# gavrissh/training-operator

Hardware: AMD Instinct MI355X
Metric: job×node fit evals/sec + gang placements/sec, 1M-node inventory, 1/2/4/8 GPUs (higher is better)
Workload: dtype int64

## Files before the change

training-operator_amd/csrc/pe_ctx.h:

```cpp
#pragma once

#include <hip/hip_runtime.h>
#include <rccl/rccl.h>

#include <immintrin.h>
#include <pthread.h>
#include <sched.h>

#include <algorithm>
#include <atomic>
#include <cstdlib>
#include <cstring>
#include <exception>
#include <functional>
#include <memory>
#include <mutex>
#include <new>
#include <stdexcept>
#include <string>
#include <thread>
#include <vector>

#include "pe_hostx.h"
#include "pe_kernels.h"
// ... 226 lines not shown
  std::thread comm_abort;
  std::unique_ptr<pe::Resolver> resolver;
  pe_allgather_fn exchange = nullptr;
  void* exchange_user = nullptr;
  void* zc_hx = nullptr;
  bool zc_ok = false;
  int topk = 256, window_groups = 112;
  bool pipeline = true;
  int64_t window_pods = 1024;
  int64_t max_nodes = 0;
  std::string gpu_name, err;
  hipStream_t stream = nullptr;
  int64_t n_total = 0, begin = 0, end = 0, Ns = 0, stride = 0;
  bool loaded = false;
  std::vector<pe::NodeState, pe::HugeAlloc<pe::NodeState>> m_nodes, m_nodes0;
  DevBuf<int64_t> res0, res;
  DevBuf<uint32_t> labels;
  DevBuf<int32_t> island;
  DevBuf<pe::NodeUpd> n_upd;
  int64_t fit_J = 0, fit_Jp = 0, Wn = 0, Wt = 0;
  bool fit_uploaded = false;
  DevBuf<ReqRec> fit_jobs;
  DevBuf<pe::ReqRec32> fit_jobs32;
  DevBuf<int32_t> res32;
  bool fit32 = false;
  int fit_shift[pe::D] = {0, 0, 0, 0};
  int fit_path = 0;
  pe::LdsSpec lds{};
  int lds_W = 4;
  int lds_shape[4] = {0, 0, 0, 0};
  int64_t lds_nblk = 0, lds_R = 1, lds_Tpad = 0, lds_npad = 0, lds_pitch = 0;
  DevBuf<pe::LdsSpec> lds_spec_d;
  DevBuf<int64_t> lds_vals;
  DevBuf<uint16_t> lds_codes;
  DevBuf<uint32_t> lds_ranks, lds_aux, lds_slots;
  DevBuf<uint32_t> lds_rows;
  int num_cu = 256;
  int fit_path_mask = PATHS_ALL;
  pe::PlaneSpec plane{};
  int64_t pl_nblk = 0;
  bool pl_rows = true;
  int64_t pl_R = 1;
  int64_t pl_pitch = 0;
  struct PlaneSet {
    pe::PlaneSpec spec;
    int64_t J, R, Jr, off;
  };
  std::vector<PlaneSet> pl_sets;
  DevBuf<pe::PlaneSpec> pl_specs_d;
  DevBuf<int64_t> pl_meta_d;
  std::vector<int64_t> pl_cnt_row;
  int64_t pl_counts_n = 0;
  DevBuf<uint32_t> planes;
  DevBuf<uint64_t> plane_jobs;
  pe::CodeSpec code{};
  int64_t code_Jp = 0, node_stride = 0;
  DevBuf<int64_t> code_vals;
  DevBuf<uint32_t> code_needs, code_jobs, code_x;
  DevBuf<uint64_t> mask;
  DevBuf<unsigned long long> counts;
  HostBuf<unsigned long long> h_counts;
  HostBuf<uint8_t> a_stage, a_outh;
  DevBuf<uint8_t> a_dstage;
  hipStream_t a_h2d = nullptr;
  std::vector<hipEvent_t> a_ev_h2d;
  HostBuf<int64_t> a_segoff;
  HostBuf<uint32_t> a_flag;
// ... 267 lines not shown
```

training-operator_amd/csrc/pe_engine.cpp:

```cpp
#include <hip/hip_runtime.h>
#include <rccl/rccl.h>

#include <immintrin.h>
#include <pthread.h>
#include <sched.h>

#include <algorithm>
#include <condition_variable>
#include <atomic>
#include <chrono>
#include <exception>
#include <functional>
#include <thread>
#include <cstdio>
#include <cstdlib>
#include <cstring>
#include <memory>
#include <mutex>
#include <new>
#include <numeric>
#include <string>
#include <unordered_map>
#include <vector>

#include "pe_ctx.h"
#include "pe_hostx.h"
#include "pe_kernels.h"
#include "pe_resolver.h"
#include "placement.h"

namespace {

double rccl_init_timeout_ms() {
  const char* e = std::getenv("PE_RCCL_INIT_TIMEOUT_S");
  const double s = e ? std::atof(e) : 120.0;
  return (s > 0 ? s : 120.0) * 1e3;
}

ncclComm_t comm_init_bounded(int device, int world, const ncclUniqueId& id, int rank, double timeout_ms) {
  struct State {
    std::mutex m;
    std::condition_variable cv;
    bool done = false, abandoned = false;
    ncclResult_t r = ncclSuccess;
    ncclComm_t comm = nullptr;
  };
  auto st = std::make_shared<State>();
  std::thread([st, device, world, id, rank] {
    (void)hipSetDevice(device);
    ncclComm_t c = nullptr;
    const ncclResult_t r = ncclCommInitRank(&c, world, id, rank);
    std::lock_guard<std::mutex> lk(st->m);
    if (st->abandoned) {
      if (r == ncclSuccess && c) (void)ncclCommDestroy(c);
      return;
    }
    st->r = r;
    st->comm = c;
    st->done = true;
    st->cv.notify_all();
// ... 1560 lines not shown
    const double t = (double)rounds * (0.02 + 1.0 / (double)r);
    if (t < best_t - 1e-9) {
      best_t = t;
      R = r;
    }
  }
  if (const char* ev = std::getenv("PE_LDS_R")) R = std::max<int64_t>(1, std::atoll(ev));
  const int64_t Tmax = ((n_jobs + R - 1) / R + 15) / 16;
  const int64_t Tpad = round_up(std::max<int64_t>(Tmax, 1), 16);
  std::vector<uint16_t> jc((size_t)n_jobs * pe::LD_CODE, 0);
  parallel_for(n_jobs, [&](int64_t j0, int64_t j1) {
  for (int64_t j = j0; j < j1; ++j) {
    uint16_t* c = jc.data() + (size_t)j * pe::LD_CODE;
    for (int i = 0; i < sp.nf; ++i) {
      const int64_t rank = (int64_t)bd.rank[fdim[i]][j] + 1;
      const int o = pe::lds_field_off(i, shape[0], shape[1], shape[2]);
      if (sp.L[i] == 1) {
        c[o] = (uint16_t)(sp.pbase[i][0] + rank - 1);
      } else {
        int64_t x = rank;
        for (int k = 0; k < sp.L[i]; ++k) {
          const int64_t digit = sp.mod[i][k] ? x % sp.mod[i][k] : x;
          x = sp.mod[i][k] ? x / sp.mod[i][k] : 0;
          c[o + k] = (uint16_t)(sp.pbase[i][k] + digit);
        }
      }
    }
    int64_t xc = 0;
    for (int x = 0; x < sp.nx; ++x) xc += (int64_t)bd.rank[fdim[sp.nf + x]][j] * sp.xstride[x];
    c[pe::lds_need_slot(shape[0], shape[1], shape[2], shape[3])] =
        (uint16_t)(sp.need_pbase + bd.rank[4][j] * sp.xprod + xc);
  }
  });
  std::vector<uint16_t> codes((size_t)(R * 16 * Tpad * pe::LD_CODE), 0);
  std::vector<uint32_t> rows((size_t)(R * 16 * Tpad), ~0u);
  {
    int64_t pos = 0;
    for (int64_t v = 0; v < R * 16; ++v) {
      const int64_t r = v / 16, w = v % 16, j0 = r + R * w;
      const int64_t T = j0 < n_jobs ? (n_jobs - j0 + 16 * R - 1) / (16 * R) : 0;
      for (int64_t t = 0; t < T; ++t, ++pos) {
        const uint32_t j = (uint32_t)(j0 + 16 * R * t);
        std::memcpy(codes.data() + (size_t)((v * Tpad + t) * pe::LD_CODE), jc.data() + (size_t)j * pe::LD_CODE,
                    pe::LD_CODE * 2);
        rows[(size_t)(v * Tpad + t)] = j;
      }
    }
    if (pos != n_jobs) raise(PE_EINVAL, "lds: run lengths do not cover the batch");
  }
  if (std::getenv("PE_LDS_DEBUG")) {
    std::fprintf(stderr, "lds: W %d nblk %lld R %lld planes %d need %d fold %d cross %d x %d |", W, (long long)nblk,
                 (long long)R, sp.nplanes, sp.nneed, sp.nfold, sp.nx, sp.xprod);
    for (int i = 0; i < sp.nf; ++i)
      std::fprintf(stderr, " dim %d m %lld L %d B %u", sp.dim[i], (long long)sp.m[i], sp.L[i], sp.mod[i][0]);
    std::fprintf(stderr, "\n");
  }
  ctx->lds = sp;
  ctx->lds_W = W;
  for (int i = 0; i < 4; ++i) ctx->lds_shape[i] = shape[i];
  ctx->lds_nblk = nblk;
  ctx->lds_R = R;
  ctx->lds_Tpad = Tpad;
  hipchk(ctx->lds_slots.ensure((size_t)R * 16 * Tpad + (size_t)ctx->lds_nblk), "alloc count slots");
  hipchk(ctx->lds_rows.ensure((size_t)R * 16 * Tpad), "alloc count rows");
  hipchk(hipMemcpyAsync(ctx->lds_rows.p, rows.data(), rows.size() * 4, hipMemcpyHostToDevice, ctx->stream),
         "H2D lds rows");
  ctx->lds_npad = nblk * S;
  ctx->lds_pitch = nblk * S / 64;
  hipchk(ctx->lds_spec_d.ensure(1), "alloc lds spec");
  hipchk(ctx->lds_vals.ensure(std::max<size_t>(allv.size(), 1)), "alloc lds vals");
  hipchk(ctx->lds_codes.ensure(codes.size()), "alloc lds codes");
  hipchk(ctx->lds_ranks.ensure((size_t)std::max(sp.nf + sp.nx, 1) * ctx->lds_npad), "alloc lds ranks");
  hipchk(ctx->lds_aux.ensure((size_t)2 * ctx->lds_npad), "alloc lds aux");
  hipchk(hipMemcpyAsync(ctx->lds_spec_d.p, &ctx->lds, sizeof(pe::LdsSpec), hipMemcpyHostToDevice, ctx->stream),
         "H2D lds spec");
  if (!allv.empty())
    hipchk(hipMemcpyAsync(ctx->lds_vals.p, allv.data(), allv.size() * 8, hipMemcpyHostToDevice, ctx->stream),
           "H2D lds vals");
  hipchk(hipMemcpyAsync(ctx->lds_codes.p, codes.data(), codes.size() * 2, hipMemcpyHostToDevice, ctx->stream),
         "H2D lds codes");
  hipchk(hipStreamSynchronize(ctx->stream), "sync lds upload");
  return true;
}

static void fit_upload(pe_ctx* ctx, int64_t n_jobs, const int64_t* req, const uint32_t* need) {
  if (n_jobs < 0) raise(PE_EINVAL, "n_jobs < 0");
  if (!ctx->loaded) raise(PE_ESTATE, "no inventory loaded");
  if (n_jobs > 0) {
    need_ptr(req, "req");
    check_req(req, n_jobs, "req");
  }
  const int64_t Jp = round_up(std::max<int64_t>(n_jobs, 1), pe::FM_JT);
  ctx->fit_J = n_jobs;
  ctx->fit_Jp = Jp;
  ctx->Wn = (ctx->Ns + 63) / 64;
  ctx->Wt = (ctx->Wn + 3) / 4;
  const bool planes_ok = ctx->fit_path_mask & PATH_PLANES;
  ctx->fit_path = -1;
  if (n_jobs > 0 && (ctx->fit_path_mask & (PATH_PLANES | PATH_LDS | PATH_CODED))) {
    BatchDict bd;
    build_dict(bd, n_jobs, req, need);
    if (planes_ok && build_planes(ctx, n_jobs, bd, false)) ctx->fit_path = 3;
    else if ((ctx->fit_path_mask & PATH_LDS) && build_lds(ctx, n_jobs, bd)) ctx->fit_path = 4;
    else if (planes_ok && build_planes(ctx, n_jobs, bd, true)) ctx->fit_path = 3;
    else if ((ctx->fit_path_mask & PATH_CODED) && build_codes(ctx, n_jobs, bd)) ctx->fit_path = 2;
  }
  if (ctx->fit_path < 0) {
    bool use32 = true;
    for (int d = 0; d < pe::D && use32; ++d) {
      int64_t mx = 0, orv = 0;
      for (int64_t j = 0; j < n_jobs; ++j) {
        mx = std::max(mx, req[j * pe::D + d]);
// ... 42 lines not shown
                                                 : (size_t)Jp * std::max<int64_t>(ctx->Wt, 1) * 4;
  static const unsigned mask_flags = std::getenv("PE_MASK_CONTIG") ? hipDeviceMallocContiguous : 0u;
  hipchk(ctx->mask.ensure(mask_words, mask_flags), "alloc fit mask");
  const int64_t n_counts = std::max<int64_t>(Jp, ctx->fit_path == 3 ? ctx->pl_counts_n : 0);
  hipchk(ctx->counts.ensure(n_counts + (ctx->fit_path == 3 ? ctx->pl_nblk : 0)), "alloc fit counts");
  hipchk(ctx->h_counts.ensure(n_counts), "alloc pinned counts");
  hipchk(hipStreamSynchronize(ctx->stream), "sync fit upload");
  ctx->fit_uploaded = true;
}

static void fit_run(pe_ctx* ctx) {
  if (!ctx->fit_uploaded) raise(PE_ESTATE, "pe_jobs_upload first");
  const int64_t J = ctx->fit_J;
  const bool encode_zeroes = ctx->fit_path == 3 && ctx->pl_sets.empty() && J > 0 && ctx->Ns > 0 && ctx->pl_nblk > 0;
  if (!encode_zeroes)
    hipchk(hipMemsetAsync(ctx->counts.p, 0, ctx->counts.n * sizeof(unsigned long long), ctx->stream), "memset counts");
  if (J == 0 || ctx->Ns == 0) return;
  const int64_t waves_y = (J + pe::FM_JT - 1) / pe::FM_JT;
  const int64_t want_x = std::max<int64_t>(1, (16384 + waves_y - 1) / waves_y);
  int64_t tpw = (ctx->Ns + 256 * want_x - 1) / (256 * want_x);
  tpw = std::min<int64_t>(16, std::max<int64_t>(1, tpw));
  if (ctx->fit_path == 4) {
    hipchk(hipMemsetAsync(ctx->lds_slots.p, 0, ((size_t)ctx->lds_R * 16 * ctx->lds_Tpad + ctx->lds_nblk) * 4, ctx->stream),
           "memset count slots");
    hipchk(pe::launch_node_ranks(ctx->stream, ctx->res.p, ctx->stride, ctx->labels.p, ctx->Ns, ctx->lds_npad,
                                 ctx->lds_spec_d.p, ctx->lds_vals.p, ctx->lds_ranks.p, ctx->lds_aux.p),
           "launch node_ranks");
    hipchk(pe::launch_fit_mask_lds(ctx->stream, ctx->lds_W, ctx->lds_shape, ctx->lds_spec_d.p, ctx->lds.nplanes,
                                   ctx->lds_ranks.p,
                                   ctx->lds_npad, ctx->lds_aux.p, ctx->lds_nblk, ctx->lds_codes.p, J,
                                   ctx->lds_R, ctx->lds_Tpad, ctx->lds_pitch * 8,
                                   reinterpret_cast<uint8_t*>(ctx->mask.p), ctx->lds_slots.p,
                                   std::getenv("PE_FIT_STATIC") ? nullptr
                                                                : ctx->lds_slots.p + (size_t)ctx->lds_R * 16 * ctx->lds_Tpad),
           "launch fit_mask_lds");
    hipchk(pe::launch_lds_counts(ctx->stream, ctx->lds_slots.p, ctx->lds_rows.p, ctx->lds_R * 16 * ctx->lds_Tpad,
                                 ctx->counts.p),
           "launch lds_counts");
    ctx->stats.fit_runs_lds += 1;
  } else if (ctx->fit_path == 3) {
    if (!ctx->pl_sets.empty()) {
      const int ns = (int)ctx->pl_sets.size();
      hipchk(pe::launch_encode_planes_sets(ctx->stream, ctx->res.p, ctx->stride, ctx->labels.p, ctx->Ns, ctx->pl_nblk,
                                           ctx->pl_specs_d.p, ns, ctx->planes.p),
             "launch encode_planes_sets");
      hipchk(pe::launch_fit_mask_planes_sets(ctx->stream, ctx->planes.p, ctx->pl_nblk, ctx->plane_jobs.p,
                                             ctx->pl_meta_d.p, ns, ctx->pl_sets[0].R,
                                             reinterpret_cast<uint32_t*>(ctx->mask.p), ctx->counts.p, ctx->pl_pitch),
             "launch fit_mask_planes_sets");
      ctx->stats.fit_runs_planes += 1;
      ctx->stats.fit_runs_sets += 1;
      ctx->stats.fit_evals += J * ctx->Ns;
      return;
    }
    hipchk(pe::launch_encode_planes(ctx->stream, ctx->res.p, ctx->stride, ctx->labels.p, ctx->Ns, ctx->pl_nblk,
                                    ctx->plane, ctx->pl_specs_d.p, ctx->planes.p, ctx->counts.p, ctx->counts.n),
           "launch encode_planes");
    if (ctx->pl_rows) {
      unsigned long long* const units = std::getenv("PE_FIT_STATIC") ? nullptr : ctx->counts.p + ctx->pl_counts_n;
      hipchk(pe::launch_fit_mask_planes_rows(ctx->stream, ctx->planes.p, ctx->pl_nblk, ctx->plane_jobs.p, J, ctx->pl_R,
                                             reinterpret_cast<uint32_t*>(ctx->mask.p), ctx->counts.p, ctx->pl_pitch,
                                             units),
             "launch fit_mask_planes_rows");
    } else {
      const int64_t ranges = std::max<int64_t>(1, (16384 + ctx->pl_nblk - 1) / ctx->pl_nblk);
      const int64_t jpw = std::max<int64_t>(64, (J + ranges - 1) / ranges);
      hipchk(pe::launch_fit_mask_planes(ctx->stream, ctx->planes.p, ctx->pl_nblk, ctx->plane_jobs.p, J, jpw,
// ... 187 lines not shown
```

training-operator_amd/csrc/pe_kernels.h:

```cpp
#pragma once
#include <hip/hip_runtime.h>
#include <stdint.h>

namespace pe {

constexpr int D = 4;
constexpr uint64_t SCORE_MAX = (1ull << 40) - 1;
constexpr uint64_t NO_KEY = ~0ull;
constexpr int64_t NEVER = INT64_MIN;

struct alignas(64) ReqRec {
  int64_t q[D];
  uint32_t need;
  uint32_t pad_[7];
};
static_assert(sizeof(ReqRec) == 64, "ReqRec must be 64 B");

struct alignas(32) ReqRec32 {
  int32_t q[D];
  uint32_t need;
  uint32_t pad_[3];
};
static_assert(sizeof(ReqRec32) == 32, "ReqRec32 must be 32 B");

// ... 133 lines not shown
constexpr int LD_NEED_SLOT = 15;
__host__ __device__ constexpr int lds_field_off(int fi, int n4, int n3, int n2) {
  return fi <= n4                ? 4 * fi
         : fi <= n4 + n3         ? 4 * n4 + 3 * (fi - n4)
         : fi <= n4 + n3 + n2    ? 4 * n4 + 3 * n3 + 2 * (fi - n4 - n3)
                                 : 4 * n4 + 3 * n3 + 2 * n2 + (fi - n4 - n3 - n2);
}
__host__ __device__ constexpr int lds_need_slot(int n4, int n3, int n2, int n1) {
  return 4 * n4 + 3 * n3 + 2 * n2 + n1;
}
constexpr int LD_THREADS = 1024;
struct LdsSpec {
  int32_t nf;
  int32_t dim[LD_MAXF];
  int32_t L[LD_MAXF];
  uint32_t div[LD_MAXF][LD_MAXL];
  uint32_t mod[LD_MAXF][LD_MAXL];
  int32_t pbase[LD_MAXF][LD_MAXL];
  int32_t vlo[LD_MAXF][LD_MAXL];
  int32_t nv[LD_MAXF][LD_MAXL];
  int32_t nneed, need_pbase, nplanes, nfold;
  int32_t nx, xprod;
  int32_t xstride[LD_MAXF];
  uint32_t needs[LD_MAXNEED];
  int32_t fold_dim[D];
  int64_t fold_val[D];
  int64_t voff[LD_MAXF];
  int64_t m[LD_MAXF];
};
hipError_t launch_node_ranks(hipStream_t s, const int64_t* res, int64_t stride, const uint32_t* labels, int64_t Ns,
                             int64_t npad, const LdsSpec* spec, const int64_t* vals, uint32_t* ranks, uint32_t* aux);
hipError_t launch_fit_mask_lds(hipStream_t s, int W, const int shape[4], const LdsSpec* spec, int nplanes,
                               const uint32_t* ranks, int64_t npad, const uint32_t* aux, int64_t nblk,
                               const uint16_t* codes, int64_t J, int64_t R, int64_t Tpad, int64_t pitch_bytes,
                               uint8_t* mask, uint32_t* slots, uint32_t* units = nullptr);
hipError_t launch_lds_counts(hipStream_t s, const uint32_t* slots, const uint32_t* rows, int64_t nslots,
                             unsigned long long* counts);

hipError_t launch_prep_nodes(hipStream_t s, const int64_t* res, int64_t stride, int64_t Ns, uint64_t id_base,
                             uint64_t* kn, uint32_t* lo );
hipError_t launch_scan(hipStream_t s, const int64_t* res, int64_t stride, const uint32_t* labels, const uint64_t* kn,
                       const uint32_t* lo, int64_t Ns, uint64_t id_base, const ReqRec* groups, int Wg, uint64_t* cand,
                       int32_t* cnt, uint64_t* bound, int nwaves);

hipError_t launch_merge(hipStream_t s, const uint64_t* cand, const int32_t* cnt, const uint64_t* bound,
                        int nwaves, int K, uint8_t* out, int Wg);

constexpr int WK_ROUND = 1024;
constexpr int WK_MAXR = 16384;
constexpr uint64_t WK_INVALID = ~0ull;
#ifndef WK_MULTI
#define WK_MULTI 2
#endif
#ifndef WK_MULTI_AFTER
#define WK_MULTI_AFTER 1
#endif
struct WalkIndex {
  uint64_t* sk;
  int64_t* sr;
  uint32_t* sl;
  uint32_t* pos;
  uint64_t* rmin;
  int64_t* rmax;
  uint32_t* ror;
  int32_t* ovl;
  int32_t* ovl_n;
  uint32_t* in_ovl;
  uint32_t* ovl_idx;
// ... 241 lines not shown
```

training-operator_amd/csrc/pe_lds.hip:

```cpp
#include "pe_lds_kernel.h"

namespace pe {

__global__ __launch_bounds__(256) void node_ranks_kernel(const int64_t* __restrict__ res, int64_t stride,
                                                         const uint32_t* __restrict__ labels, int64_t Ns, int64_t npad,
                                                         const LdsSpec* __restrict__ spp,
                                                         const int64_t* __restrict__ vals, uint32_t* __restrict__ ranks,
                                                         uint32_t* __restrict__ aux) {
  const LdsSpec& sp = *spp;
  const int64_t n = (int64_t)blockIdx.x * blockDim.x + threadIdx.x;
  if (n >= npad) return;
  const bool real = n < Ns;
  uint32_t ok = real ? 1u : 0u;
  for (int i = 0; i < sp.nfold; ++i) ok &= real && res[sp.fold_dim[i] * stride + n] >= sp.fold_val[i];
  aux[n] = ok;
  aux[npad + n] = real ? labels[n] : 0u;
  for (int f = 0; f < sp.nf + sp.nx; ++f) {
    uint32_t R = 0;
    if (real) {
      const int64_t x = res[sp.dim[f] * stride + n];
      const int64_t* v = vals + sp.voff[f];
      int64_t lo = 0, hi = sp.m[f];
      while (lo < hi) {
        const int64_t mid = (lo + hi) >> 1;
        if (v[mid] <= x) lo = mid + 1;
        else hi = mid;
      }
      R = (uint32_t)lo;
    }
    ranks[f * npad + n] = R;
  }
}

hipError_t launch_node_ranks(hipStream_t s, const int64_t* res, int64_t stride, const uint32_t* labels, int64_t Ns,
                             int64_t npad, const LdsSpec* spec, const int64_t* vals, uint32_t* ranks, uint32_t* aux) {
  if (npad <= 0) return hipSuccess;
  hipLaunchKernelGGL(node_ranks_kernel, dim3((unsigned)((npad + 255) / 256)), dim3(256), 0, s, res, stride, labels, Ns,
                     npad, spec, vals, ranks, aux);
  return hipGetLastError();
}

hipError_t launch_fit_mask_lds(hipStream_t s, int W, const int shape[4], const LdsSpec* spec, int nplanes,
                               const uint32_t* ranks, int64_t npad, const uint32_t* aux, int64_t nblk,
                               const uint16_t* codes, int64_t J, int64_t R, int64_t Tpad, int64_t pitch_bytes,
                               uint8_t* mask, uint32_t* slots, uint32_t* units) {
  if (J <= 0 || nblk <= 0 || R <= 0) return hipSuccess;
  const size_t lds = (size_t)nplanes * 2048 * W / 8;
  if (lds > 160 * 1024) return hipErrorInvalidValue;
  const void* fn = W == 1   ? lds_kernel_w1(shape[0], shape[1], shape[2], shape[3])
                   : W == 2 ? lds_kernel_w2(shape[0], shape[1], shape[2], shape[3])
                   : W == 4 ? lds_kernel_w4(shape[0], shape[1], shape[2], shape[3])
                            : nullptr;
  if (!fn) return hipErrorInvalidValue;
  hipError_t e = hipFuncSetAttribute(fn, hipFuncAttributeMaxDynamicSharedMemorySize, (int)lds);
  if (e != hipSuccess) return e;
  const uint2* c = reinterpret_cast<const uint2*>(codes);
  void* args[] = {(void*)&spec, (void*)&ranks, (void*)&npad, (void*)&aux,         (void*)&nblk,   (void*)&c,
                  (void*)&J,    (void*)&R,     (void*)&Tpad, (void*)&pitch_bytes, (void*)&mask,   (void*)&slots,
                  (void*)&units};
  e = hipLaunchKernel(fn, dim3((unsigned)(nblk * R)), dim3(LD_THREADS), args, lds, s);
  if (e != hipSuccess) return e;
  return hipGetLastError();
}

__global__ __launch_bounds__(256) void lds_counts_kernel(const uint32_t* __restrict__ slots,
                                                         const uint32_t* __restrict__ rows, int64_t nslots,
                                                         unsigned long long* __restrict__ counts) {
  const int64_t s = (int64_t)blockIdx.x * blockDim.x + threadIdx.x;
  if (s >= nslots) return;
  const uint32_t j = rows[s];
  if (j != ~0u) counts[j] = slots[s];
}

hipError_t launch_lds_counts(hipStream_t s, const uint32_t* slots, const uint32_t* rows, int64_t nslots,
                             unsigned long long* counts) {
  if (nslots <= 0) return hipSuccess;
  hipLaunchKernelGGL(lds_counts_kernel, dim3((unsigned)((nslots + 255) / 256)), dim3(256), 0, s, slots, rows, nslots,
                     counts);
  return hipGetLastError();
}

}
```

training-operator_amd/csrc/pe_lds_kernel.h:

```cpp
#pragma once
#include "pe_kernels.h"
#include "pe_wave.h"

namespace pe {

template <int W> struct LdVec;
template <> struct LdVec<1> { typedef uint32_t T; };
template <> struct LdVec<2> { typedef uint32_t T __attribute__((ext_vector_type(2))); };
template <> struct LdVec<4> { typedef uint32_t T __attribute__((ext_vector_type(4))); };

template <int W>
__device__ __forceinline__ uint32_t popc_vec(typename LdVec<W>::T v) {
  if constexpr (W == 1) return __popc(v);
  else if constexpr (W == 2) return __popc(v.x) + __popc(v.y);
  else return __popc(v.x) + __popc(v.y) + __popc(v.z) + __popc(v.w);
}

template <int W>
__device__ __forceinline__ void slice_split(typename LdVec<W>::T v, uint32_t (&o)[W]) {
  if constexpr (W == 1) o[0] = v;
  else {
#pragma unroll
    for (int i = 0; i < W; ++i) o[i] = v[i];
  }
}
template <int W>
__device__ __forceinline__ typename LdVec<W>::T slice_join(const uint32_t (&o)[W]) {
  typename LdVec<W>::T v;
  if constexpr (W == 1) v = o[0];
  else {
#pragma unroll
    for (int i = 0; i < W; ++i) v[i] = o[i];
  }
  return v;
}

template <int W>
__device__ __forceinline__ typename LdVec<W>::T plane_rd(const uint32_t* lds, uint32_t p, int lane) {
  return *reinterpret_cast<const typename LdVec<W>::T*>(lds + p * (64u * W) + (uint32_t)lane * W);
}

template <int W, int N4, int N3, int N2, int N1>
__global__ __launch_bounds__(LD_THREADS) void fit_mask_lds_kernel(const LdsSpec* __restrict__ spp,
                                                                  const uint32_t* __restrict__ ranks, int64_t npad,
                                                                  const uint32_t* __restrict__ aux, int64_t nblk,
                                                                  const uint2* __restrict__ codes, int64_t J,
                                                                  int64_t R, int64_t Tpad, int64_t pitch_bytes,
                                                                  uint8_t* __restrict__ mask,
                                                                  uint32_t* __restrict__ slots,
                                                                  uint32_t* __restrict__ units) {
  typedef typename LdVec<W>::T V;
  constexpr int S = 2048 * W;
  constexpr int WPP = S / 32;
  extern __shared__ uint32_t lds[];
  const LdsSpec& sp = *spp;
  const int tid = threadIdx.x, lane = tid & 63;
  const int wave = __builtin_amdgcn_readfirstlane(tid >> 6);
  const int64_t blk = blockIdx.x % nblk, r = blockIdx.x / nblk;
  const int64_t n0 = blk * S;

  const int ndig = sp.need_pbase * WPP;
  for (int i = tid; i < ndig; i += LD_THREADS) lds[i] = 0u;
  __syncthreads();
  int cols = 0;
  for (int f = 0; f < sp.nf; ++f) cols += sp.L[f] * WPP;
  for (int c = tid; c < cols; c += LD_THREADS) {
    int f = 0, rest = c;
    while (rest >= sp.L[f] * WPP) rest -= sp.L[f++] * WPP;
    const int k = rest / WPP, w = rest % WPP;
    const uint32_t* rk = ranks + f * npad + n0 + 32 * w;
    const uint32_t dv = sp.div[f][k], md = sp.mod[f][k];
    const int vlo = sp.vlo[f][k], nv = sp.nv[f][k];
    uint32_t* const base = lds + sp.pbase[f][k] * WPP + w;
    for (int b = 0; b < 32; ++b) {
      uint32_t d = rk[b] / dv;
      if (md) d %= md;
      const int v = (int)d - vlo;
      if (v >= 0 && v < nv) base[v * WPP] |= 1u << b;
    }
  }
  __syncthreads();
  for (int c = tid; c < cols; c += LD_THREADS) {
    int f = 0, rest = c;
    while (rest >= sp.L[f] * WPP) rest -= sp.L[f++] * WPP;
    const int k = rest / WPP, w = rest % WPP;
    uint32_t* const base = lds + sp.pbase[f][k] * WPP + w;
// ... 1 lines not shown
    for (int v = sp.nv[f][k] - 1; v >= 0; --v) {
      acc |= base[v * WPP];
      base[v * WPP] = acc;
    }
  }
  for (int g = wave; g < S / 64; g += LD_THREADS / 64) {
    const int64_t n = n0 + 64 * g + lane;
    const bool ok = aux[n] != 0u;
    const uint32_t lab = aux[npad + n];
    uint32_t xr[LD_MAXF];
#pragma unroll
    for (int x = 0; x < LD_MAXF; ++x) xr[x] = x < sp.nx ? ranks[(sp.nf + x) * npad + n] : 0u;
    for (int i = 0; i < sp.nneed; ++i) {
      const bool li = ok && (lab & sp.needs[i]) == sp.needs[i];
      uint32_t dig[LD_MAXF] = {0u, 0u, 0u, 0u};
      for (int c = 0; c < sp.xprod; ++c) {
        bool pass = li;
#pragma unroll
        for (int x = 0; x < LD_MAXF; ++x) pass = pass && (x >= sp.nx || xr[x] > dig[x]);
        const uint64_t b = __ballot(pass);
        if (lane == 0) *reinterpret_cast<uint64_t*>(lds + (sp.need_pbase + i * sp.xprod + c) * WPP + 2 * g) = b;
        bool carry = true;
#pragma unroll
        for (int x = 0; x < LD_MAXF; ++x)
          if (carry && x < sp.nx) {
            carry = ++dig[x] == (uint32_t)sp.m[sp.nf + x];
            if (carry) dig[x] = 0u;
          }
      }
    }
  }
  __syncthreads();

  const int64_t step = 16 * R;
  auto runT = [&](int64_t q) -> int64_t {
    const int64_t j0q = q / 16 + R * (q % 16);
    return j0q < J ? (J - j0q + step - 1) / step : 0;
  };
  const int64_t nq = R * 16;
  const int64_t nbt = (runT(0) + 15) / 16;
  const int64_t Ulast = units ? nq * nbt : (runT(r * 16 + wave) + 15) / 16;
  uint8_t* const col0 = mask + blk * (S / 8);
  const uint32_t lane_off = (uint32_t)lane * (4 * W);
  uint32_t sigma;
  {
    uint32_t probe[16];
#pragma unroll
    for (int k = 0; k < 16; ++k) probe[k] = lane == 0 ? (uint32_t)k : 0u;
    sigma = reduce16x64(probe, lane);
  }
  auto run_of = [&](int64_t u) -> int64_t { return units ? u % nq : r * 16 + wave; };
  auto batch_of = [&](int64_t u) -> int64_t { return units ? u / nq : u; };
  int64_t st = 0;
  auto grab = [&]() -> int64_t {
    if (!units) return st++;
    uint32_t v = 0;
    if (lane == 0) v = atomicAdd(units + blk, 1u);
    return (int64_t)v;
  };
  auto codes_of = [&](int64_t u) -> uint2 {
    const int64_t q = u < Ulast ? run_of(u) : 0, t0 = u < Ulast ? 16 * batch_of(u) : 0;
    return codes[q * Tpad * (LD_CODE / 4) + min<int64_t>(t0, Tpad - 16) * (LD_CODE / 4) + lane];
  };
  int64_t u0 = __builtin_amdgcn_readfirstlane((int)grab());
  int64_t u1v = grab();
  uint2 cv = codes_of(u0);
  asm volatile("" : : "v"(cv.x), "v"(cv.y));
  while (u0 < Ulast) {
    const int64_t u1 = __builtin_amdgcn_readfirstlane((int)u1v);
    const int64_t u2v = grab();
    const int64_t q = run_of(u0), t0 = 16 * batch_of(u0), T = runT(q);
    const int64_t j0 = q / 16 + R * (q % 16);
    uint32_t* const sl = slots + q * Tpad;
    const int n = __builtin_amdgcn_readfirstlane((int)max<int64_t>(0, min<int64_t>(16, T - t0)));
    const uint2 cur = cv;
    cv = codes_of(u1);
    uint32_t p[16];
#pragma unroll
    for (int K = 0; K < 16; ++K) {
      const int64_t j = j0 + step * (t0 + K);
      auto entry = [&](int e) -> uint32_t {
        const uint32_t d = (uint32_t)__builtin_amdgcn_readlane((int)((e & 2) ? cur.y : cur.x), 4 * K + e / 4);
        return (e & 1) ? d >> 16 : d & 0xFFFFu;
      };
      uint32_t f[W];
      slice_split<W>(plane_rd<W>(lds, entry(lds_need_slot(N4, N3, N2, N1)), lane), f);
#pragma unroll
      for (int fi = 0; fi < N4 + N3 + N2 + N1; ++fi) {
        const int L = fi < N4 ? 4 : fi < N4 + N3 ? 3 : fi < N4 + N3 + N2 ? 2 : 1;
        const int o = lds_field_off(fi, N4, N3, N2);
        uint32_t a[W], g[W], h[W];
        slice_split<W>(plane_rd<W>(lds, entry(o), lane), a);
#pragma unroll
        for (int k = 1; k < L; ++k) {
          const uint32_t pk = entry(o + k);
#ifdef PE_LDS_OPAQUE_PAIR
          uint32_t ph = pk + 1;
          if constexpr (W == 2) asm("" : "+s"(ph));
          slice_split<W>(plane_rd<W>(lds, pk, lane), g);
          slice_split<W>(plane_rd<W>(lds, ph, lane), h);
#else
          slice_split<W>(plane_rd<W>(lds, pk, lane), g);
          if constexpr (W == 2) __builtin_amdgcn_sched_barrier(0x7FF);
          slice_split<W>(plane_rd<W>(lds, pk + 1, lane), h);
#endif
#pragma unroll
          for (int i = 0; i < W; ++i) a[i] = h[i] | (g[i] & a[i]);
        }
#pragma unroll
        for (int i = 0; i < W; ++i) f[i] &= a[i];
      }
      const V fv = slice_join<W>(f);
      const __amdgpu_buffer_rsrc_t rs =
          __builtin_amdgcn_make_buffer_rsrc((void*)(col0 + j * pitch_bytes), 0, K < n ? 256 * W : 0, 0x00020000);
      if constexpr (W == 1) __builtin_amdgcn_raw_buffer_store_b32(fv, rs, lane_off, 0, 0);
      else if constexpr (W == 2) __builtin_amdgcn_raw_buffer_store_b64(fv, rs, lane_off, 0, 0);
      else __builtin_amdgcn_raw_buffer_store_b128(fv, rs, lane_off, 0, 0);
      p[K] = popc_vec<W>(fv);
    }
    const uint32_t F = reduce16x64(p, lane);
    if ((lane & 3) == 0 && sigma < (uint32_t)n && F) atomicAdd(&sl[t0 + sigma], F);
    u0 = u1;
    u1v = u2v;
  }
}

#define PE_LDS_SHAPES3(X, W)                                                                             \
  X(W, 0, 0, 0, 0) X(W, 0, 0, 0, 1) X(W, 0, 0, 0, 2) X(W, 0, 0, 0, 3) X(W, 0, 0, 0, 4) X(W, 0, 0, 1, 0)  \
  X(W, 0, 0, 1, 1) X(W, 0, 0, 1, 2) X(W, 0, 0, 1, 3) X(W, 0, 0, 2, 0) X(W, 0, 0, 2, 1) X(W, 0, 0, 2, 2)  \
  X(W, 0, 0, 3, 0) X(W, 0, 0, 3, 1) X(W, 0, 0, 4, 0) X(W, 0, 1, 0, 0) X(W, 0, 1, 0, 1) X(W, 0, 1, 0, 2)  \
  X(W, 0, 1, 0, 3) X(W, 0, 1, 1, 0) X(W, 0, 1, 1, 1) X(W, 0, 1, 1, 2) X(W, 0, 1, 2, 0) X(W, 0, 1, 2, 1)  \
  X(W, 0, 1, 3, 0) X(W, 0, 2, 0, 0) X(W, 0, 2, 0, 1) X(W, 0, 2, 0, 2) X(W, 0, 2, 1, 0) X(W, 0, 2, 1, 1)  \
  X(W, 0, 2, 2, 0) X(W, 0, 3, 0, 0) X(W, 0, 3, 0, 1) X(W, 0, 3, 1, 0) X(W, 0, 4, 0, 0)

#define PE_LDS_SHAPES4(X, W)                                                                             \
  X(W, 1, 0, 0, 0) X(W, 1, 0, 0, 1) X(W, 1, 0, 0, 2) X(W, 1, 0, 0, 3) X(W, 1, 0, 1, 0) X(W, 1, 0, 1, 1)  \
  X(W, 1, 0, 1, 2) X(W, 1, 0, 2, 0) X(W, 1, 0, 2, 1) X(W, 1, 0, 3, 0) X(W, 1, 1, 0, 0) X(W, 1, 1, 0, 1)  \
  X(W, 1, 1, 0, 2) X(W, 1, 1, 1, 0) X(W, 1, 1, 1, 1) X(W, 1, 1, 2, 0) X(W, 1, 2, 0, 0) X(W, 1, 2, 0, 1)  \
  X(W, 1, 2, 1, 0) X(W, 1, 3, 0, 0) X(W, 2, 0, 0, 0) X(W, 2, 0, 0, 1) X(W, 2, 0, 0, 2) X(W, 2, 0, 1, 0)  \
  X(W, 2, 0, 1, 1) X(W, 2, 0, 2, 0) X(W, 2, 1, 0, 0) X(W, 2, 1, 0, 1) X(W, 2, 1, 1, 0) X(W, 2, 2, 0, 0)  \
  X(W, 3, 0, 0, 0) X(W, 3, 0, 0, 1) X(W, 3, 0, 1, 0) X(W, 3, 1, 0, 0)

template <int W>
const void* lds_kernel_for(int n4, int n3, int n2, int n1) {
#define PE_LDS_PICK(W_, a, b, c, d) \
  if (n4 == a && n3 == b && n2 == c && n1 == d) return (const void*)fit_mask_lds_kernel<W_, a, b, c, d>;
  PE_LDS_SHAPES3(PE_LDS_PICK, W)
  if constexpr (W >= 2) {
    PE_LDS_SHAPES4(PE_LDS_PICK, W)
  }
#undef PE_LDS_PICK
  return nullptr;
}

const void* lds_kernel_w1(int n4, int n3, int n2, int n1);
const void* lds_kernel_w2(int n4, int n3, int n2, int n1);
// ... 4 lines not shown
```

Before: 46670 billion.

## Pre-encode LDS byte offsets in job codes and specialize full-batch store path

Job codes are now uploaded as 32-bit words holding precomputed LDS byte offsets for two planes each, so the kernel masks an offset and ORs in the lane offset instead of multiplying plane indices. The main loop moves from 64-bit to 32-bit index arithmetic, and full 16-job batches take a fast path that issues buffer stores through a scalar row-stride offset, with no per-job resource rebuilds or bounds-limited descriptors. Partial batches fall back to a simple loop with wave reductions. This is meant to cut scalar and vector address overhead in the inner fit loop, at the cost of a wider code upload and new size limits on J, R and the stride.

Result: no change. 46610 billion (-0.1%).

```diff
diff --git a/training-operator_amd/csrc/pe_ctx.h b/training-operator_amd/csrc/pe_ctx.h
--- a/training-operator_amd/csrc/pe_ctx.h
+++ b/training-operator_amd/csrc/pe_ctx.h
@@ -282,7 +282,7 @@
   int64_t lds_nblk = 0, lds_R = 1, lds_Tpad = 0, lds_npad = 0, lds_pitch = 0;
   DevBuf<pe::LdsSpec> lds_spec_d;
   DevBuf<int64_t> lds_vals;
-  DevBuf<uint16_t> lds_codes;
+  DevBuf<uint32_t> lds_codes;
   DevBuf<uint32_t> lds_ranks, lds_aux, lds_slots;
   DevBuf<uint32_t> lds_rows;
   int num_cu = 256;
diff --git a/training-operator_amd/csrc/pe_engine.cpp b/training-operator_amd/csrc/pe_engine.cpp
--- a/training-operator_amd/csrc/pe_engine.cpp
+++ b/training-operator_amd/csrc/pe_engine.cpp
@@ -26,6 +26,7 @@
 #include "pe_ctx.h"
 #include "pe_hostx.h"
 #include "pe_kernels.h"
+#include "pe_lds_code.h"
 #include "pe_resolver.h"
 #include "placement.h"
 
@@ -1652,7 +1653,8 @@
         (uint16_t)(sp.need_pbase + bd.rank[4][j] * sp.xprod + xc);
   }
   });
-  std::vector<uint16_t> codes((size_t)(R * 16 * Tpad * pe::LD_CODE), 0);
+  constexpr int CW = pe::LD_CODE / 2;
+  std::vector<uint32_t> codes((size_t)(R * 16 * Tpad * CW), 0);
   std::vector<uint32_t> rows((size_t)(R * 16 * Tpad), ~0u);
   {
     int64_t pos = 0;
@@ -1661,8 +1663,14 @@
       const int64_t T = j0 < n_jobs ? (n_jobs - j0 + 16 * R - 1) / (16 * R) : 0;
       for (int64_t t = 0; t < T; ++t, ++pos) {
         const uint32_t j = (uint32_t)(j0 + 16 * R * t);
-        std::memcpy(codes.data() + (size_t)((v * Tpad + t) * pe::LD_CODE), jc.data() + (size_t)j * pe::LD_CODE,
-                    pe::LD_CODE * 2);
+        const uint16_t* c = jc.data() + (size_t)j * pe::LD_CODE;
+        uint32_t* out = codes.data() + (size_t)((v * Tpad + t) * CW);
+        for (int d = 0; d < CW; ++d) {
+          uint32_t even = 0, odd = 0;
+          if (!pe::lds_plane_off(c[2 * d], W, &even) || !pe::lds_plane_off(c[2 * d + 1], W, &odd))
+            raise(PE_EINVAL, "lds: a job's plane lies outside the block image");
+          out[d] = pe::lds_code_pack(even, odd);
+        }
         rows[(size_t)(v * Tpad + t)] = j;
       }
     }
@@ -1697,7 +1705,7 @@
   if (!allv.empty())
     hipchk(hipMemcpyAsync(ctx->lds_vals.p, allv.data(), allv.size() * 8, hipMemcpyHostToDevice, ctx->stream),
            "H2D lds vals");
-  hipchk(hipMemcpyAsync(ctx->lds_codes.p, codes.data(), codes.size() * 2, hipMemcpyHostToDevice, ctx->stream),
+  hipchk(hipMemcpyAsync(ctx->lds_codes.p, codes.data(), codes.size() * 4, hipMemcpyHostToDevice, ctx->stream),
          "H2D lds codes");
   hipchk(hipStreamSynchronize(ctx->stream), "sync lds upload");
   return true;
@@ -1806,7 +1814,8 @@
                                    ctx->lds_R, ctx->lds_Tpad, ctx->lds_pitch * 8,
                                    reinterpret_cast<uint8_t*>(ctx->mask.p), ctx->lds_slots.p,
                                    std::getenv("PE_FIT_STATIC") ? nullptr
-                                                                : ctx->lds_slots.p + (size_t)ctx->lds_R * 16 * ctx->lds_Tpad),
+                                                                : ctx->lds_slots.p + (size_t)ctx->lds_R * 16 * ctx->lds_Tpad,
+                                   std::getenv("PE_LDS_ROWS64") != nullptr),
            "launch fit_mask_lds");
     hipchk(pe::launch_lds_counts(ctx->stream, ctx->lds_slots.p, ctx->lds_rows.p, ctx->lds_R * 16 * ctx->lds_Tpad,
                                  ctx->counts.p),
diff --git a/training-operator_amd/csrc/pe_kernels.h b/training-operator_amd/csrc/pe_kernels.h
--- a/training-operator_amd/csrc/pe_kernels.h
+++ b/training-operator_amd/csrc/pe_kernels.h
@@ -189,8 +189,9 @@
                              int64_t npad, const LdsSpec* spec, const int64_t* vals, uint32_t* ranks, uint32_t* aux);
 hipError_t launch_fit_mask_lds(hipStream_t s, int W, const int shape[4], const LdsSpec* spec, int nplanes,
                                const uint32_t* ranks, int64_t npad, const uint32_t* aux, int64_t nblk,
-                               const uint16_t* codes, int64_t J, int64_t R, int64_t Tpad, int64_t pitch_bytes,
-                               uint8_t* mask, uint32_t* slots, uint32_t* units = nullptr);
+                               const uint32_t* codes, int64_t J, int64_t R, int64_t Tpad, int64_t pitch_bytes,
+                               uint8_t* mask, uint32_t* slots, uint32_t* units = nullptr,
+                               bool rows64 = false);
 hipError_t launch_lds_counts(hipStream_t s, const uint32_t* slots, const uint32_t* rows, int64_t nslots,
                              unsigned long long* counts);
 
diff --git a/training-operator_amd/csrc/pe_lds.hip b/training-operator_amd/csrc/pe_lds.hip
--- a/training-operator_amd/csrc/pe_lds.hip
+++ b/training-operator_amd/csrc/pe_lds.hip
@@ -42,11 +42,13 @@
 
 hipError_t launch_fit_mask_lds(hipStream_t s, int W, const int shape[4], const LdsSpec* spec, int nplanes,
                                const uint32_t* ranks, int64_t npad, const uint32_t* aux, int64_t nblk,
-                               const uint16_t* codes, int64_t J, int64_t R, int64_t Tpad, int64_t pitch_bytes,
-                               uint8_t* mask, uint32_t* slots, uint32_t* units) {
+                               const uint32_t* codes, int64_t J, int64_t R, int64_t Tpad, int64_t pitch_bytes,
+                               uint8_t* mask, uint32_t* slots, uint32_t* units, bool rows64) {
   if (J <= 0 || nblk <= 0 || R <= 0) return hipSuccess;
   const size_t lds = (size_t)nplanes * 2048 * W / 8;
-  if (lds > 160 * 1024) return hipErrorInvalidValue;
+  if (lds > LD_LDS_BYTES) return hipErrorInvalidValue;
+  if (J >= (int64_t(1) << 30) || R >= (int64_t(1) << 20) || Tpad < 16) return hipErrorInvalidValue;
+  uint32_t stride32 = rows64 ? 0u : lds_row_stride32(R, pitch_bytes);
   const void* fn = W == 1   ? lds_kernel_w1(shape[0], shape[1], shape[2], shape[3])
                    : W == 2 ? lds_kernel_w2(shape[0], shape[1], shape[2], shape[3])
                    : W == 4 ? lds_kernel_w4(shape[0], shape[1], shape[2], shape[3])
@@ -54,10 +56,14 @@
   if (!fn) return hipErrorInvalidValue;
   hipError_t e = hipFuncSetAttribute(fn, hipFuncAttributeMaxDynamicSharedMemorySize, (int)lds);
   if (e != hipSuccess) return e;
+  hipFuncAttributes fa;
+  e = hipFuncGetAttributes(&fa, fn);
+  if (e != hipSuccess) return e;
+  if (fa.sharedSizeBytes != 0) return hipErrorInvalidValue;
   const uint2* c = reinterpret_cast<const uint2*>(codes);
   void* args[] = {(void*)&spec, (void*)&ranks, (void*)&npad, (void*)&aux,         (void*)&nblk,   (void*)&c,
                   (void*)&J,    (void*)&R,     (void*)&Tpad, (void*)&pitch_bytes, (void*)&mask,   (void*)&slots,
-                  (void*)&units};
+                  (void*)&units, (void*)&stride32};
   e = hipLaunchKernel(fn, dim3((unsigned)(nblk * R)), dim3(LD_THREADS), args, lds, s);
   if (e != hipSuccess) return e;
   return hipGetLastError();
diff --git a/training-operator_amd/csrc/pe_lds_code.h b/training-operator_amd/csrc/pe_lds_code.h
--- /dev/null
+++ b/training-operator_amd/csrc/pe_lds_code.h
@@ -0,0 +1,38 @@
+#pragma once
+#include <stdint.h>
+
+#if defined(__HIP_DEVICE_COMPILE__)
+#define PE_LC_HD __host__ __device__ __forceinline__
+#elif defined(__HIPCC__)
+#define PE_LC_HD __host__ __device__ inline
+#else
+#define PE_LC_HD inline
+#endif
+
+namespace pe {
+
+constexpr uint32_t LD_OFF_MASK = 0x3FF00u;
+constexpr int LD_ODD_SHIFT = 14;
+constexpr uint32_t LD_LDS_BYTES = 160 * 1024;
+
+PE_LC_HD bool lds_plane_off(uint32_t p, int W, uint32_t* off) {
+  const uint64_t o = (uint64_t)p * 256u * (uint32_t)W;
+  if (o + 256u * (uint32_t)W > LD_LDS_BYTES) return false;
+  *off = (uint32_t)o;
+  return true;
+}
+
+PE_LC_HD uint32_t lds_code_pack(uint32_t off_even, uint32_t off_odd) { return off_even | off_odd << LD_ODD_SHIFT; }
+PE_LC_HD uint32_t lds_code_even(uint32_t dword) { return dword & LD_OFF_MASK; }
+PE_LC_HD uint32_t lds_code_odd(uint32_t dword) { return (dword >> LD_ODD_SHIFT) & LD_OFF_MASK; }
+
+PE_LC_HD uint32_t lds_row_stride32(int64_t R, int64_t pitch_bytes) {
+  if (R <= 0 || pitch_bytes <= 0) return 0;
+  const uint64_t lim = uint64_t(1) << 32;
+  if ((uint64_t)R >= lim / 256 || (uint64_t)pitch_bytes >= lim) return 0;
+  const uint64_t stride = 16u * (uint64_t)R * (uint64_t)pitch_bytes;
+  if (stride * 16u >= lim) return 0;
+  return (uint32_t)stride;
+}
+
+}
diff --git a/training-operator_amd/csrc/pe_lds_kernel.h b/training-operator_amd/csrc/pe_lds_kernel.h
--- a/training-operator_amd/csrc/pe_lds_kernel.h
+++ b/training-operator_amd/csrc/pe_lds_kernel.h
@@ -1,5 +1,6 @@
 #pragma once
 #include "pe_kernels.h"
+#include "pe_lds_code.h"
 #include "pe_wave.h"
 
 namespace pe {
@@ -33,11 +34,6 @@
     for (int i = 0; i < W; ++i) v[i] = o[i];
   }
   return v;
-}
-
-template <int W>
-__device__ __forceinline__ typename LdVec<W>::T plane_rd(const uint32_t* lds, uint32_t p, int lane) {
-  return *reinterpret_cast<const typename LdVec<W>::T*>(lds + p * (64u * W) + (uint32_t)lane * W);
 }
 
 template <int W, int N4, int N3, int N2, int N1>
@@ -48,10 +44,11 @@
                                                                   int64_t R, int64_t Tpad, int64_t pitch_bytes,
                                                                   uint8_t* __restrict__ mask,
                                                                   uint32_t* __restrict__ slots,
-                                                                  uint32_t* __restrict__ units) {
+                                                                  uint32_t* __restrict__ units, uint32_t stride32) {
   typedef typename LdVec<W>::T V;
   constexpr int S = 2048 * W;
   constexpr int WPP = S / 32;
+  constexpr int READS = 1 + 7 * N4 + 5 * N3 + 3 * N2 + N1;
   extern __shared__ uint32_t lds[];
   const LdsSpec& sp = *spp;
   const int tid = threadIdx.x, lane = tid & 63;
@@ -119,14 +116,13 @@
   }
   __syncthreads();
 
-  const int64_t step = 16 * R;
-  auto runT = [&](int64_t q) -> int64_t {
-    const int64_t j0q = q / 16 + R * (q % 16);
-    return j0q < J ? (J - j0q + step - 1) / step : 0;
-  };
-  const int64_t nq = R * 16;
-  const int64_t nbt = (runT(0) + 15) / 16;
-  const int64_t Ulast = units ? nq * nbt : (runT(r * 16 + wave) + 15) / 16;
+  const uint32_t nq = 16u * (uint32_t)R;
+  const uint32_t Ta = (uint32_t)J / nq, Trem = (uint32_t)J % nq;
+  auto run_j0 = [&](uint32_t q) -> uint32_t { return (q >> 4) + (uint32_t)R * (q & 15u); };
+  auto runT = [&](uint32_t q) -> uint32_t { return Ta + (run_j0(q) < Trem ? 1u : 0u); };
+  const uint32_t q_own = (uint32_t)r * 16u + (uint32_t)wave;
+  const uint32_t nbt = (runT(0) + 15u) / 16u;
+  const uint32_t Ulast = units ? nq * nbt : (runT(q_own) + 15u) / 16u;
   uint8_t* const col0 = mask + blk * (S / 8);
   const uint32_t lane_off = (uint32_t)lane * (4 * W);
   uint32_t sigma;
@@ -136,79 +132,141 @@
     for (int k = 0; k < 16; ++k) probe[k] = lane == 0 ? (uint32_t)k : 0u;
     sigma = reduce16x64(probe, lane);
   }
-  auto run_of = [&](int64_t u) -> int64_t { return units ? u % nq : r * 16 + wave; };
-  auto batch_of = [&](int64_t u) -> int64_t { return units ? u / nq : u; };
-  int64_t st = 0;
-  auto grab = [&]() -> int64_t {
-    if (!units) return st++;
-    uint32_t v = 0;
-    if (lane == 0) v = atomicAdd(units + blk, 1u);
-    return (int64_t)v;
-  };
-  auto codes_of = [&](int64_t u) -> uint2 {
-    const int64_t q = u < Ulast ? run_of(u) : 0, t0 = u < Ulast ? 16 * batch_of(u) : 0;
-    return codes[q * Tpad * (LD_CODE / 4) + min<int64_t>(t0, Tpad - 16) * (LD_CODE / 4) + lane];
-  };
-  int64_t u0 = __builtin_amdgcn_readfirstlane((int)grab());
-  int64_t u1v = grab();
-  uint2 cv = codes_of(u0);
-  asm volatile("" : : "v"(cv.x), "v"(cv.y));
+  uint32_t st = 0;
+  uint32_t ctr_idx = 0u;
+#ifndef PE_LDS_GRAB_UNIFORM
+  asm("" : "+v"(ctr_idx));
+#endif
+  auto grab = [&]() -> uint32_t {
+    uint32_t v = st++;
+    if (units && lane == 0) v = atomicAdd(units + blk + ctr_idx, 1u);
+    return v;
+  };
+  auto first = [&](uint32_t v) -> uint32_t { return (uint32_t)__builtin_amdgcn_readfirstlane((int)v); };
+  auto unit = [&](uint32_t u, uint32_t& q, uint32_t& t0) {
+    if (u >= Ulast) {
+      q = 0u;
+      t0 = 0u;
+    } else if (units) {
+      const uint32_t b = u / nq;
+      q = u - b * nq;
+      t0 = 16u * b;
+    } else {
+      q = q_own;
+      t0 = 16u * u;
+    }
+  };
+  auto codes_of = [&](uint32_t q, uint32_t t0) -> uint2 {
+    return codes[((int64_t)q * Tpad + min(t0, (uint32_t)Tpad - 16u)) * (LD_CODE / 4) + lane];
+  };
+  uint32_t off_mask = LD_OFF_MASK;
+  asm volatile("" : "+v"(off_mask));
+  auto job = [&](uint32_t cx, uint32_t cy, int K4) -> V {
+    auto addr = [&](int e) -> uint32_t {
+      const uint32_t d = (uint32_t)__builtin_amdgcn_readlane((int)((e & 2) ? cy : cx), K4 + e / 4);
+      return (((e & 1) ? d >> LD_ODD_SHIFT : d) & off_mask) | lane_off;
+    };
+    auto rd = [&](uint32_t a) -> V {
+      typedef const V __attribute__((address_space(3))) * LdsPtr;
+      return *(LdsPtr)(size_t)a;
+    };
+    uint32_t f[W];
+    slice_split<W>(rd(addr(lds_need_slot(N4, N3, N2, N1))), f);
+#pragma unroll
+    for (int fi = 0; fi < N4 + N3 + N2 + N1; ++fi) {
+      const int L = fi < N4 ? 4 : fi < N4 + N3 ? 3 : fi < N4 + N3 + N2 ? 2 : 1;
+      const int o = lds_field_off(fi, N4, N3, N2);
+      uint32_t a[W], g[W], h[W];
+      slice_split<W>(rd(addr(o)), a);
+#pragma unroll
+      for (int k = 1; k < L; ++k) {
+        const uint32_t pk = addr(o + k);
+#ifdef PE_LDS_OPAQUE_PAIR
+        uint32_t ph = pk + 256 * W;
+        if constexpr (W == 2) asm("" : "+v"(ph));
+        slice_split<W>(rd(pk), g);
+        slice_split<W>(rd(ph), h);
+#else
+        slice_split<W>(rd(pk), g);
+        if constexpr (W == 2) __builtin_amdgcn_sched_barrier(0x7FF);
+        slice_split<W>(rd(pk + 256 * W), h);
+#endif
+#pragma unroll
+        for (int i = 0; i < W; ++i) a[i] = h[i] | (g[i] & a[i]);
+      }
+#pragma unroll
+      for (int i = 0; i < W; ++i) f[i] &= a[i];
+      if constexpr (W * READS > 64) __builtin_amdgcn_sched_barrier(0);
+    }
+    return slice_join<W>(f);
+  };
+  uint32_t u0 = first(grab());
+  uint32_t u1v = grab();
+  uint32_t q, t0;
+  unit(u0, q, t0);
+  auto landed = [&](uint2 c, uint32_t& u) -> uint2 {
+    uint2 o;
+    uint32_t uo;
+    asm volatile("v_mov_b32 %0, %3\n\tv_mov_b32 %1, %4\n\tv_mov_b32 %2, %5"
+                 : "=&v"(o.x), "=&v"(o.y), "=&v"(uo)
+                 : "v"(c.x), "v"(c.y), "v"(u));
+    u = uo;
+    return o;
+  };
+  uint2 cur = landed(codes_of(q, t0), u1v);
   while (u0 < Ulast) {
-    const int64_t u1 = __builtin_amdgcn_readfirstlane((int)u1v);
-    const int64_t u2v = grab();
-    const int64_t q = run_of(u0), t0 = 16 * batch_of(u0), T = runT(q);
-    const int64_t j0 = q / 16 + R * (q % 16);
-    uint32_t* const sl = slots + q * Tpad;
-    const int n = __builtin_amdgcn_readfirstlane((int)max<int64_t>(0, min<int64_t>(16, T - t0)));
-    const uint2 cur = cv;
-    cv = codes_of(u1);
-    uint32_t p[16];
-#pragma unroll
-    for (int K = 0; K < 16; ++K) {
-      const int64_t j = j0 + step * (t0 + K);
-      auto entry = [&](int e) -> uint32_t {
-        const uint32_t d = (uint32_t)__builtin_amdgcn_readlane((int)((e & 2) ? cur.y : cur.x), 4 * K + e / 4);
-        return (e & 1) ? d >> 16 : d & 0xFFFFu;
-      };
-      uint32_t f[W];
-      slice_split<W>(plane_rd<W>(lds, entry(lds_need_slot(N4, N3, N2, N1)), lane), f);
-#pragma unroll
-      for (int fi = 0; fi < N4 + N3 + N2 + N1; ++fi) {
-        const int L = fi < N4 ? 4 : fi < N4 + N3 ? 3 : fi < N4 + N3 + N2 ? 2 : 1;
-        const int o = lds_field_off(fi, N4, N3, N2);
-        uint32_t a[W], g[W], h[W];
-        slice_split<W>(plane_rd<W>(lds, entry(o), lane), a);
-#pragma unroll
-        for (int k = 1; k < L; ++k) {
-          const uint32_t pk = entry(o + k);
-#ifdef PE_LDS_OPAQUE_PAIR
-          uint32_t ph = pk + 1;
-          if constexpr (W == 2) asm("" : "+s"(ph));
-          slice_split<W>(plane_rd<W>(lds, pk, lane), g);
-          slice_split<W>(plane_rd<W>(lds, ph, lane), h);
-#else
-          slice_split<W>(plane_rd<W>(lds, pk, lane), g);
-          if constexpr (W == 2) __builtin_amdgcn_sched_barrier(0x7FF);
-          slice_split<W>(plane_rd<W>(lds, pk + 1, lane), h);
-#endif
-#pragma unroll
-          for (int i = 0; i < W; ++i) a[i] = h[i] | (g[i] & a[i]);
+    const uint32_t u1 = first(u1v);
+    const uint32_t T = runT(q);
+    uint32_t* const sl = slots + (int64_t)q * Tpad + t0;
+    uint8_t* const row0 = col0 + ((int64_t)run_j0(q) + (int64_t)nq * t0) * pitch_bytes;
+    const uint32_t n = T > t0 ? min(16u, T - t0) : 0u;
+    uint32_t q1, t1;
+    unit(u1, q1, t1);
+    uint32_t u2v;
+    uint2 nxt;
+    if (n == 16u && stride32 != 0u) {
+      u2v = grab();
+      const uint2 cv = codes_of(q1, t1);
+      __builtin_amdgcn_sched_barrier(0);
+      const __amdgpu_buffer_rsrc_t rs = __builtin_amdgcn_make_buffer_rsrc((void*)row0, 0, -1, 0x00020000);
+      uint32_t soff = 0u;
+      uint32_t p[16];
+#pragma unroll
+      for (int K = 0; K < 16; ++K) {
+        const V fv = job(cur.x, cur.y, 4 * K);
+        if constexpr (W == 1) __builtin_amdgcn_raw_buffer_store_b32(fv, rs, lane_off, soff, 0);
+        else if constexpr (W == 2) __builtin_amdgcn_raw_buffer_store_b64(fv, rs, lane_off, soff, 0);
+        else {
+          const __amdgpu_buffer_rsrc_t rk =
+              __builtin_amdgcn_make_buffer_rsrc((void*)(row0 + soff), 0, -1, 0x00020000);
+          __builtin_amdgcn_raw_buffer_store_b128(fv, rk, lane_off, 0, 0);
         }
-#pragma unroll
-        for (int i = 0; i < W; ++i) f[i] &= a[i];
+        p[K] = popc_vec<W>(fv);
+        soff += stride32;
+        asm("" : "+s"(soff));
       }
-      const V fv = slice_join<W>(f);
-      const __amdgpu_buffer_rsrc_t rs =
-          __builtin_amdgcn_make_buffer_rsrc((void*)(col0 + j * pitch_bytes), 0, K < n ? 256 * W : 0, 0x00020000);
-      if constexpr (W == 1) __builtin_amdgcn_raw_buffer_store_b32(fv, rs, lane_off, 0, 0);
-      else if constexpr (W == 2) __builtin_amdgcn_raw_buffer_store_b64(fv, rs, lane_off, 0, 0);
-      else __builtin_amdgcn_raw_buffer_store_b128(fv, rs, lane_off, 0, 0);
-      p[K] = popc_vec<W>(fv);
-    }
-    const uint32_t F = reduce16x64(p, lane);
-    if ((lane & 3) == 0 && sigma < (uint32_t)n && F) atomicAdd(&sl[t0 + sigma], F);
+      nxt = landed(cv, u2v);
+      const uint32_t F = reduce16x64(p, lane);
+      if ((lane & 3) == 0 && F) atomicAdd(&sl[sigma], F);
+    } else {
+      uint32_t acc = 0u;
+      for (uint32_t K = 0; K < n; ++K) {
+        const V fv = job(cur.x, cur.y, (int)(4u * K));
+        *reinterpret_cast<V*>(row0 + (int64_t)K * nq * pitch_bytes + lane_off) = fv;
+        uint32_t c = popc_vec<W>(fv);
+#pragma unroll
+        for (int o = 32; o > 0; o >>= 1) c += __shfl_xor(c, o, 64);
+        if ((uint32_t)lane == K) acc = c;
+      }
+      if (acc) atomicAdd(&sl[lane], acc);
+      u2v = grab();
+      nxt = landed(codes_of(q1, t1), u2v);
+    }
+    cur = nxt;
     u0 = u1;
     u1v = u2v;
+    q = q1;
+    t0 = t1;
   }
 }
 
```
